# e4s2024/E4S2024

Measured on AMD Instinct MI355X. Metric: 1024x1024 faces/sec (StyleGAN2 regional synthesis, gen_img), higher is better.
Workload: dtype f16+mxfp6x2 (masked 3x3 layers >= 32^2) / bf16x3 (all other layers); 1 GPU; BASELINE configs[1]: StyleGAN2 1024x1024 synthesis from random W+, 12-region masks, batch=4/GPU; batch_per_gpu=4, global_batch=4, parallelism=frames x1, streams_per_gpu=2

## Files before the change

e4s2024_amd/csrc/modconv_upblock_mx.hip:

```cpp
#include "modconv_mx_tile.h"

#ifndef UX_ABL
#define UX_ABL 0
#endif
#ifndef UX_BACK
#define UX_BACK 0
#endif

namespace {

constexpr int UX_OUT = 16;
constexpr int UX_TN = 64, UX_CK = 32;
constexpr int UX_T = UX_OUT / 2 + 2;
constexpr int UX_PW = UX_T + 1;
constexpr int UX_PATCH = UX_PW * UX_PW;
constexpr int UX_NPOS = UX_T * UX_T;
constexpr int UX_EST = 128;
constexpr int UX_ZR = 2 * UX_T, UX_ZS = UX_ZR + 2;
constexpr int UX_NUNIT = 5;
constexpr int UX_U_W16 = 2 * 2 * 2 * UX_TN * 16;
constexpr int UX_U_CLO = 2 * 2 * UX_TN * 16;
constexpr int UX_U_CHI = 2 * 2 * UX_TN * 8;
constexpr int UX_U_SC = 2 * UX_TN * 4;
constexpr int UX_UNITB = 15 * 1024;
constexpr int UX_NPIECE = UX_UNITB / 1024;
static_assert(UX_U_W16 + UX_U_CLO + UX_U_CHI + UX_U_SC <= UX_UNITB, "unit slot");
constexpr int UX_NSLOT = 6;
constexpr int UX_RING = 0;
constexpr int UX_GRP0 = UX_RING + UX_NSLOT * UX_UNITB;
constexpr int UX_A1 = 0;
constexpr int UX_CLO = UX_A1 + 4 * UX_EST * 16;
constexpr int UX_CHI = UX_CLO + 2 * UX_EST * 16;
constexpr int UX_SC = UX_CHI + 2 * UX_EST * 8;
constexpr int UX_SROW = UX_SC + UX_EST * 4;
constexpr int UX_MAX_CIN = 512;
constexpr int UX_EP = UX_SROW + UX_MAX_CIN * 4;
constexpr int UX_RAW = UX_EP + (2 * UX_TN + UX_OUT * UX_OUT) * 4;
constexpr int UX_GRPB = UX_RAW + UX_CK * UX_EST * 4;
constexpr int UX_LDS = UX_GRP0 + 2 * UX_GRPB;
constexpr int UX_ZTB = 16 * UX_ZR * UX_ZS * 4;
static_assert(UX_LDS <= 160 * 1024 && 2 * UX_ZTB <= UX_GRP0 && UX_GRPB % 16 == 0, "LDS plan; the pre-blur tiles overlay the weight ring");

struct UpBlockMxParams {
    float* out;
    const float* x;
    const unsigned char* wmx;
    const float* s;
    const float* d;
    const uint8_t* blocks;
    const int* ctrl;
    const float* blur;
    const float* noise;
    const float* noise_weight;
    const float* act_bias;
    int* flags;
    int noise_bstride, act;
    int bs, cin, cout, h, w, nreg;
    int nbx, nby;
    unsigned perm_mul;
};

__device__ __forceinline__ void ux_wait_vm(int n) {
    switch (n) {
#define UX_CASE(v) case v: E4S_WAIT_VM(v); break;
        UX_CASE(0) UX_CASE(1) UX_CASE(2) UX_CASE(3) UX_CASE(4) UX_CASE(5) UX_CASE(6) UX_CASE(8) UX_CASE(10)
        UX_CASE(16) UX_CASE(17) UX_CASE(18) UX_CASE(19) UX_CASE(20) UX_CASE(21) UX_CASE(22) UX_CASE(24) UX_CASE(26)
        UX_CASE(32) UX_CASE(33) UX_CASE(34) UX_CASE(35) UX_CASE(36) UX_CASE(38) UX_CASE(40)
#undef UX_CASE
        default: E4S_WAIT_VM(0); break;
    }
}

__host__ __device__ constexpr int ux_tap_ky(int u, int d) { return u == 0 ? 0 : u == 1 ? 2 : u == 2 ? 1 : u == 3 ? (d ? 2 : 0) : (d ? 3 : 1); }
__host__ __device__ constexpr int ux_tap_kx(int u, int d) { return u == 0 ? (d ? 2 : 0) : u == 1 ? (d ? 2 : 0) : u == 2 ? (d ? 2 : 0) : 1; }
__host__ __device__ constexpr int ux_parity(int u) { return u == 0 ? 0 : u == 1 ? 0 : u == 2 ? 2 : u == 3 ? 1 : 3; }

__global__ __launch_bounds__(256) void prep_weights_upblock_mx_kernel(unsigned char* __restrict__ dst, const float* __restrict__ weight, int cout, int cin, float scale) {
    const int nchunk = cin / UX_CK, ntile = (cout + UX_TN - 1) / UX_TN;
    const int64_t total = (int64_t)nchunk * ntile * UX_NUNIT * 2 * UX_TN;
    for (int64_t i = (int64_t)blockIdx.x * 256 + threadIdx.x; i < total; i += (int64_t)gridDim.x * 256) {
        int64_t r = i;
        const int n = (int)(r % UX_TN); r /= UX_TN;
        const int half = (int)(r & 1); r >>= 1;
        const int unit = (int)(r % UX_NUNIT); r /= UX_NUNIT;
        const int tile = (int)(r % ntile);
        const int chunk = (int)(r / ntile);
        const int co = tile * UX_TN + n;
        const int ky = ux_tap_ky(unit, half), kx = ux_tap_kx(unit, half);
        unsigned char* slot = dst + (((size_t)chunk * ntile + tile) * UX_NUNIT + unit) * UX_UNITB;
        u32x16 q1, q2;
        float m1 = 0.f, m2 = 0.f;
#pragma unroll
        for (int j = 0; j < 16; ++j) {
            float a = 0.f, b = 0.f;
            if (ky < 3 && co < cout) {
                a = weight[((size_t)co * cin + chunk * UX_CK + 2 * j) * 9 + ky * 3 + kx] * scale;
                b = weight[((size_t)co * cin + chunk * UX_CK + 2 * j + 1) * 9 + ky * 3 + kx] * scale;
            }
            const f16x2 hh = __builtin_convertvector((f32x2){a, b}, f16x2);
            const float ra = (a - (float)hh[0]) * 4096.f, rb = (b - (float)hh[1]) * 4096.f;
            q1[j] = __builtin_bit_cast(unsigned, hh);
            q2[j] = pack_f16_rne(ra, rb);
            m1 = fmaxf(m1, fmaxf(fabsf((float)hh[0]), fabsf((float)hh[1])));
            m2 = fmaxf(m2, fmaxf(fabsf(ra), fabsf(rb)));
        }
        uint4* w16 = reinterpret_cast<uint4*>(slot);
#pragma unroll
        for (int s = 0; s < 4; ++s) w16[(half * 4 + s) * UX_TN + n] = make_uint4(q1[4 * s], q1[4 * s + 1], q1[4 * s + 2], q1[4 * s + 3]);
        auto expo = [](float m) { const unsigned ex = (__builtin_bit_cast(unsigned, m) >> 23) & 0xffu; return ex > 3u ? ex - 2u : 1u; };
        const unsigned e1 = expo(m1), e2 = expo(m2);
        const u32x6 c1 = __builtin_amdgcn_cvt_scalef32_pk32_fp6_f16(__builtin_bit_cast(f16x32, q1), __builtin_bit_cast(float, e1 << 23));
        const u32x6 c2 = __builtin_amdgcn_cvt_scalef32_pk32_fp6_f16(__builtin_bit_cast(f16x32, q2), __builtin_bit_cast(float, e2 << 23));
        uint4* clo = reinterpret_cast<uint4*>(slot + UX_U_W16);
        uint2* chi = reinterpret_cast<uint2*>(slot + UX_U_W16 + UX_U_CLO);
        unsigned* scp = reinterpret_cast<unsigned*>(slot + UX_U_W16 + UX_U_CLO + UX_U_CHI);
        clo[(0 * 2 + half) * UX_TN + n] = make_uint4(c1[0], c1[1], c1[2], c1[3]);
        chi[(0 * 2 + half) * UX_TN + n] = make_uint2(c1[4], c1[5]);
        clo[(1 * 2 + half) * UX_TN + n] = make_uint4(c2[0], c2[1], c2[2], c2[3]);
        chi[(1 * 2 + half) * UX_TN + n] = make_uint2(c2[4], c2[5]);
        const unsigned e2s = e2 > 12u ? e2 - 12u : 0u;
        scp[half * UX_TN + n] = e1 | (e2s << 8);
    }
}

__global__ __launch_bounds__(512, 2) void masked_up_block_mx_kernel(const UpBlockMxParams p) {
    const int npx = p.nbx >> 1;
    const int pr_i = (int)(((unsigned long long)blockIdx.x * p.perm_mul) % gridDim.x);
    const int tyt = pr_i / npx, txp = pr_i - tyt * npx;
    const int b = blockIdx.z;
    if (p.ctrl[2] == 0) return;
    const int reg_a = p.blocks[((size_t)b * p.nby + tyt) * p.nbx + 2 * txp], reg_b = p.blocks[((size_t)b * p.nby + tyt) * p.nbx + 2 * txp + 1];
    if (reg_a >= p.nreg && reg_b >= p.nreg) return;

    extern __shared__ __attribute__((aligned(16))) unsigned char lds[];
    const int tid = threadIdx.x;
    const int lane = tid & 63;
    const int wave = __builtin_amdgcn_readfirstlane(tid >> 6);
    const int grp = wave >> 2, gw = wave & 3;
    const int lt = tid & 255;
    const int txt = 2 * txp + grp;
    const int reg = grp ? reg_b : reg_a;
    const bool live = reg < p.nreg;
    unsigned char* gl = lds + UX_GRP0 + grp * UX_GRPB;
    const int l5 = lane & 31, khalf = lane >> 5;
    const int cot = blockIdx.y, co0 = cot * UX_TN;
    const int ncot = (p.cout + UX_TN - 1) / UX_TN;
    const int hw = p.h * p.w, ho = 2 * p.h, wo = 2 * p.w;
    const int nchunk = p.cin / UX_CK, nunits = nchunk * UX_NUNIT;
    const float* xb = p.x + (size_t)b * p.cin * hw;

    const unsigned char* wbase = p.wmx + (size_t)cot * UX_NUNIT * UX_UNITB;
    auto dma_unit = [&](int g, int slot) __attribute__((always_inline)) {
        const int chunk = g / UX_NUNIT, u = g - chunk * UX_NUNIT;
        const unsigned char* src = wbase + ((size_t)chunk * ncot * UX_NUNIT + u) * UX_UNITB;
#pragma unroll
        for (int k = 0; k < 2; ++k) {
            const int piece = wave + 8 * k;
            if (piece < UX_NPIECE) dma16_asm(src + piece * 1024, (unsigned)(lane * 16), (unsigned)(UX_RING + slot * UX_UNITB + piece * 1024));
        }
    };

    const int pt = (gw & 1) * 64 + lane;
#if UX_BACK & 1
    const bool has_x = gw < 2 && live, has_cv = has_x;
    constexpr int LD_NC = UX_CK;
    const int ld_c0 = 0;
#else
    const bool has_x = live, has_cv = live && (gw >> 1) == grp;
    constexpr int LD_NC = UX_CK / 2;
    const int ld_c0 = (gw >> 1) * LD_NC;
#endif
    const int PCS = wave < 7 ? 2 : 1;
    const int NLD = has_x ? LD_NC : 0;
    auto patch_pixel = [&](bool& in) __attribute__((always_inline)) {
        int t = pt;
        pin_here(t);
        const int se_y = t / UX_PW, se_x = t - se_y * UX_PW;
        const int sgy = tyt * (UX_OUT / 2) - 2 + se_y, sgx = txt * (UX_OUT / 2) - 2 + se_x;
        in = t < UX_PATCH && sgy >= 0 && sgy < p.h && sgx >= 0 && sgx < p.w;
        return in ? (unsigned)(sgy * p.w + sgx) * 4u : 0u;
    };
    const unsigned raw_dst = (unsigned)(UX_GRP0 + grp * UX_GRPB + UX_RAW + (gw & 1) * 64 * 4);
    auto load_x = [&](int chunk) __attribute__((always_inline)) {
        if (has_x) {
            bool in;
            const unsigned goff = patch_pixel(in);
#pragma unroll
            for (int c = 0; c < LD_NC; ++c) dma4_asm(xb + (size_t)(chunk * UX_CK + ld_c0 + c) * hw, goff, raw_dst + (unsigned)((ld_c0 + c) * UX_EST * 4));
        }
    };
    unsigned ovf = 0u;
    auto store_x = [&](int chunk) __attribute__((always_inline)) {
        if (!has_cv) return;
        bool in;
        (void)patch_pixel(in);
        const float4* st = reinterpret_cast<const float4*>(gl + UX_SROW) + chunk * (UX_CK / 4);
        float xr[UX_CK];
        {
            int t = pt;
            pin_here(t);
            const float* raw = reinterpret_cast<const float*>(gl + UX_RAW) + t;
#pragma unroll
            for (int c = 0; c < UX_CK; ++c) xr[c] = raw[c * UX_EST];
        }
        u32x16 q1, q2;
        unsigned m = 0u;
#pragma unroll
        for (int half = 0; half < 2; ++half) {
            float4 s4[4];
#pragma unroll
            for (int k = 0; k < 4; ++k) s4[k] = st[half * 4 + k];
#pragma unroll
            for (int k = 0; k < 4; ++k) {
                const int c4 = half * 4 + k;
                const float a0 = xr[4 * c4] * s4[k].x, a1v = xr[4 * c4 + 1] * s4[k].y, a2v = xr[4 * c4 + 2] * s4[k].z, a3 = xr[4 * c4 + 3] * s4[k].w;
                q1[2 * c4] = pack_f16_rne(a0, a1v);
                q1[2 * c4 + 1] = pack_f16_rne(a2v, a3);
                q2[2 * c4] = resid_pair_f16(xr[4 * c4], s4[k].x, xr[4 * c4 + 1], s4[k].y, q1[2 * c4]);
                q2[2 * c4 + 1] = resid_pair_f16(xr[4 * c4 + 2], s4[k].z, xr[4 * c4 + 3], s4[k].w, q1[2 * c4 + 1]);
                typedef unsigned short u16x2 __attribute__((ext_vector_type(2)));
                u16x2 mm = __builtin_elementwise_max(__builtin_bit_cast(u16x2, m), __builtin_bit_cast(u16x2, q1[2 * c4] & 0x7fff7fffu));
                mm = __builtin_elementwise_max(mm, __builtin_bit_cast(u16x2, q1[2 * c4 + 1] & 0x7fff7fffu));
                m = __builtin_bit_cast(unsigned, mm);
            }
        }
        if (!in) {
#pragma unroll
            for (int j = 0; j < 16; ++j) { q1[j] = 0u; q2[j] = 0u; }
            m = 0u;
        }
        const unsigned mh = (m & 0xffffu) > (m >> 16) ? (m & 0xffffu) : (m >> 16);
        const unsigned e16 = mh >> 10;
        ovf |= e16 >= 31u ? 1u : 0u;
        const unsigned ex = (e16 ? e16 : 1u) + 112u;
        const unsigned e1 = ex > 3u ? ex - 2u : 1u, e2 = ex > 14u ? ex - 13u : 1u;
        const u32x6 c1 = __builtin_amdgcn_cvt_scalef32_pk32_fp6_f16(__builtin_bit_cast(f16x32, q1), __builtin_bit_cast(float, e1 << 23));
        const u32x6 c2 = __builtin_amdgcn_cvt_scalef32_pk32_fp6_f16(__builtin_bit_cast(f16x32, q2), __builtin_bit_cast(float, e2 << 23));
        int t = pt;
        pin_here(t);
        if (t < UX_PATCH) {
            uint4* a1p = reinterpret_cast<uint4*>(gl + UX_A1);
#pragma unroll
            for (int s = 0; s < 4; ++s) a1p[s * UX_EST + t] = make_uint4(q1[4 * s], q1[4 * s + 1], q1[4 * s + 2], q1[4 * s + 3]);
            uint4* clo = reinterpret_cast<uint4*>(gl + UX_CLO);
            uint2* chi = reinterpret_cast<uint2*>(gl + UX_CHI);
            clo[t] = make_uint4(c1[0], c1[1], c1[2], c1[3]);
            chi[t] = make_uint2(c1[4], c1[5]);
            clo[UX_EST + t] = make_uint4(c2[0], c2[1], c2[2], c2[3]);
            chi[UX_EST + t] = make_uint2(c2[4], c2[5]);
            reinterpret_cast<unsigned*>(gl + UX_SC)[t] = e1 | (e2 << 8);
        }
    };

    if (live) {
        const float* srow = p.s + ((size_t)b * p.nreg + reg) * p.cin;
        float* sl = reinterpret_cast<float*>(gl + UX_SROW);
        for (int c = lt; c < p.cin; c += 256) sl[c] = srow[c];
        float* ep_d = reinterpret_cast<float*>(gl + UX_EP);
        float* ep_b = ep_d + UX_TN;
        float* ep_n = ep_b + UX_TN;
        if (lt < UX_TN) {
            const int co = co0 + lt;
            ep_d[lt] = (co < p.cout && p.d) ? p.d[((size_t)b * p.nreg + reg) * p.cout + co] : 1.f;
            ep_b[lt] = (co < p.cout && p.act_bias) ? p.act_bias[co] : 0.f;
        }
        {
            const int ny = tyt * UX_OUT + (lt >> 4), nx = txt * UX_OUT + (lt & 15);
            ep_n[lt] = (p.noise && ny < ho && nx < wo) ? p.noise_weight[0] * p.noise[(size_t)b * p.noise_bstride + (size_t)ny * wo + nx] : 0.f;
        }
    }
    load_x(0);
#pragma unroll
    for (int k = 0; k < UX_NSLOT; ++k)
        if (k < nunits) dma_unit(k, k);
    ux_wait_vm(((nunits < UX_NSLOT ? nunits : UX_NSLOT) - 1) * PCS);
    E4S_LDS_BARRIER();
    store_x(0);
    E4S_LDS_BARRIER();

#if UX_BACK & 2
    const int pos = gw * 32 + l5;
    const bool pos_ok = pos < UX_NPOS;
    const int posc = pos_ok ? pos : UX_NPOS - 1;
    const int pty = posc / UX_T, ptx = posc - pty * UX_T;
    const int xoff = pty * UX_PW + ptx;
#else
    const int lq = l5 >> 2;
    const int li = l5 - 4 * ((lq + 1) >> 1);
    const int lr = li == 15 ? 0 : li / 5, lc = li == 15 ? 5 : li - 5 * lr;
    const int pty = 3 * gw + lr, ptx = 5 * ((0x96 >> lq) & 1) + lc;
    const bool pos_ok = li < 15 && pty < UX_T;
    const int xoff = pty * UX_PW + ptx - (pty >= UX_T ? 32 : 0);
#endif

    f32x16 accs[4][2];
#pragma unroll
    for (int a = 0; a < 4; ++a)
#pragma unroll
        for (int i = 0; i < 2; ++i)
#pragma unroll
            for (int r = 0; r < 16; ++r) accs[a][i][r] = 0.f;

    const unsigned char* wl = lds + UX_RING + (khalf * UX_TN + l5) * 16;
    uint4 xa[2][2], wv[2][2][2];
    auto tap_entry = [&](int u, int d) __attribute__((always_inline)) {
        int xo = xoff;
        pin_here(xo);
        return xo + (1 - (ux_tap_ky(u, d) >> 1)) * UX_PW + (1 - (ux_tap_kx(u, d) >> 1));
    };
    auto read_f16 = [&](int u, int d, int slot) __attribute__((always_inline)) {
        const unsigned char* ws = wl + slot * UX_UNITB;
        const int e = tap_entry(u, d);
#pragma unroll
        for (int j = 0; j < 2; ++j) {
            xa[d][j] = *reinterpret_cast<const uint4*>(gl + UX_A1 + ((2 * j + khalf) * UX_EST + e) * 16);
#pragma unroll
            for (int cb = 0; cb < 2; ++cb) wv[cb][d][j] = *reinterpret_cast<const uint4*>(ws + ((d * 2 + j) * 2 * UX_TN + cb * 32) * 16);
        }
    };
    auto mfma_f16 = [&](int ai, int d) __attribute__((always_inline)) {
#pragma unroll
        for (int j = 0; j < 2; ++j)
#pragma unroll
            for (int cb = 0; cb < 2; ++cb)
                accs[ai][cb] = __builtin_amdgcn_mfma_f32_32x32x16_f16(__builtin_bit_cast(f16x8, wv[cb][d][j]), __builtin_bit_cast(f16x8, xa[d][j]), accs[ai][cb], 0, 0, 0);
    };
    int slot = 0, g = 0;
    if (!(UX_ABL & 1)) read_f16(0, 0, 0);
#pragma unroll 1
    for (int chunk = 0; chunk < ((UX_ABL & 1) ? 0 : nchunk); ++chunk) {
        const bool more = chunk + 1 < nchunk;
        if (more && !(UX_ABL & 4)) load_x(chunk + 1);
#pragma unroll
        for (int u = 0; u < UX_NUNIT; ++u, ++g) {
            const int ai = ux_parity(u);
            const int nslot = slot == UX_NSLOT - 1 ? 0 : slot + 1;
            const bool two = u < UX_NUNIT - 1;
            uint4 calo[2], wclo[2][2];
            uint2 cahi[2], wchi[2][2];
            int scw[2], sca = 0;
            auto read_fp6 = [&](int term) __attribute__((always_inline)) {
                const int ek = (khalf && two) ? tap_entry(u, 1) : tap_entry(u, 0);
                calo[term] = *reinterpret_cast<const uint4*>(gl + UX_CLO + (term * UX_EST + ek) * 16);
                cahi[term] = *reinterpret_cast<const uint2*>(gl + UX_CHI + (term * UX_EST + ek) * 8);
                const unsigned char* wc = lds + UX_RING + slot * UX_UNITB + UX_U_W16 + (khalf * UX_TN + l5) * 16;
                const unsigned char* wh = lds + UX_RING + slot * UX_UNITB + UX_U_W16 + UX_U_CLO + (khalf * UX_TN + l5) * 8;
#pragma unroll
                for (int cb = 0; cb < 2; ++cb) {
                    wclo[cb][1 - term] = *reinterpret_cast<const uint4*>(wc + ((1 - term) * 2 * UX_TN + cb * 32) * 16);
                    wchi[cb][1 - term] = *reinterpret_cast<const uint2*>(wh + ((1 - term) * 2 * UX_TN + cb * 32) * 8);
                }
                if (term == 0) {
                    sca = *reinterpret_cast<const int*>(gl + UX_SC + ek * 4);
                    const unsigned char* wsc = lds + UX_RING + slot * UX_UNITB + UX_U_W16 + UX_U_CLO + UX_U_CHI + (khalf * UX_TN + l5) * 4;
#pragma unroll
                    for (int cb = 0; cb < 2; ++cb) scw[cb] = *reinterpret_cast<const int*>(wsc + cb * 32 * 4);
                }
            };
            if (two) read_f16(u, 1, slot);
            __builtin_amdgcn_sched_barrier(0);
            if (live) mfma_f16(ai, 0);
            __builtin_amdgcn_sched_barrier(0);
            read_fp6(0);
            __builtin_amdgcn_sched_barrier(0);
            if (live && two) mfma_f16(ai, 1);
            __builtin_amdgcn_sched_barrier(0);
            read_fp6(1);
            __builtin_amdgcn_sched_barrier(0);
            if (live) {
#pragma unroll
                for (int cb = 0; cb < 2; ++cb)
                    accs[ai][cb] = __builtin_amdgcn_mfma_scale_f32_32x32x64_f8f6f4(mx_op6(wclo[cb][1], wchi[cb][1]), mx_op6(calo[0], cahi[0]), accs[ai][cb], 2, 2, 1, scw[cb], 0, sca);
            }
            __builtin_amdgcn_sched_barrier(0);
            {
                const int last_req = g - 1 + UX_NSLOT < nunits - 1 ? g - 1 + UX_NSLOT : nunits - 1;
                const int younger = last_req > g + 1 ? last_req - (g + 1) : 0;
                const bool addx = u < UX_NUNIT - 1 && more && !(UX_ABL & 4) && NLD != 0;
                if (younger == UX_NSLOT - 2 && LD_NC == 16) {
                    static_assert(UX_NSLOT == 6, "the literals below are 4 units of 2 / 1 pieces + 16 activation requests");
                    if (addx) { if (PCS == 2) E4S_WAIT_VM(24); else E4S_WAIT_VM(20); }
                    else { if (PCS == 2) E4S_WAIT_VM(8); else E4S_WAIT_VM(4); }
                } else
                    ux_wait_vm(younger * PCS + (addx ? NLD : 0));
            }
            E4S_LDS_BARRIER();
            if (g + UX_NSLOT < nunits) dma_unit(g + UX_NSLOT, slot);
            if (two) {
                read_f16(u + 1, 0, nslot);
                __builtin_amdgcn_sched_barrier(0);
            }
            if (live) {
#pragma unroll
                for (int cb = 0; cb < 2; ++cb)
                    accs[ai][cb] = __builtin_amdgcn_mfma_scale_f32_32x32x64_f8f6f4(mx_op6(wclo[cb][0], wchi[cb][0]), mx_op6(calo[1], cahi[1]), accs[ai][cb], 2, 2, 0, scw[cb], 1, sca);
            }
            slot = nslot;
        }
        if (more) {
            if (!(UX_ABL & 4)) store_x(chunk + 1);
            E4S_LDS_BARRIER();
            read_f16(0, 0, slot);
        }
    }
    E4S_WAIT_VM(0);
    if (p.flags && __builtin_amdgcn_ballot_w64(ovf != 0u) != 0 && lane == 0) { atomicOr(p.flags, 1); atomicAdd(p.flags + 1, 1); }

    if (UX_ABL & 2) { if (accs[0][0][0] == 12345.f) p.out[tid] = accs[1][1][1] + accs[2][0][2] + accs[3][1][3]; return; }
    __syncthreads();
    float* zt = reinterpret_cast<float*>(lds + grp * UX_ZTB);
    const float* ep_d = reinterpret_cast<const float*>(gl + UX_EP);
    const float* ep_b = ep_d + UX_TN;
    const float* ep_n = ep_b + UX_TN;
    float kf[16];
#pragma unroll
    for (int t = 0; t < 16; ++t) kf[t] = p.blur[15 - t];
    const int bx = lt & 15, bco = (lt >> 4) & 7, byg = (lt >> 7) & 1;
    const int oy0 = tyt * UX_OUT + 8 * byg, ox = txt * UX_OUT + bx;
    int nrow = ho - oy0;
    nrow = (!live || nrow < 0) ? 0 : (nrow > 8 ? 8 : nrow);
    const bool col_ok = ox < wo;
    const float* nzp = ep_n + 8 * byg * UX_OUT + bx;
    float nzr[8];
#pragma unroll
    for (int r = 0; r < 8; ++r) nzr[r] = nzp[r * UX_OUT];
    const float neg = p.act ? 0.2f : 1.f, gain = p.act ? 1.41421356237309515f : 1.f;
#pragma unroll
    for (int i = 0; i < 2; ++i) {
#pragma unroll
        for (int gh = 0; gh < 2; ++gh) {
            if (pos_ok && live) {
#pragma unroll
                for (int g2 = 0; g2 < 2; ++g2)
#pragma unroll
                    for (int rr = 0; rr < 4; ++rr) {
                        const int col = 8 * g2 + 4 * khalf + rr;
#pragma unroll
                        for (int ci = 0; ci < 2; ++ci)
                            *reinterpret_cast<float2*>(&zt[(col * UX_ZR + 2 * pty + ci) * UX_ZS + 2 * ptx]) =
                                make_float2(accs[2 * ci][i][4 * (2 * gh + g2) + rr], accs[2 * ci + 1][i][4 * (2 * gh + g2) + rr]);
                    }
            }
            __syncthreads();
            if (nrow > 0 && col_ok) {
#pragma unroll
                for (int c2 = 0; c2 < 2; ++c2) {
                    const int lc = bco + 8 * c2;
                    const int cl = i * 32 + 16 * gh + lc;
                    const int co = co0 + cl;
                    if (co >= p.cout) continue;
                    const float dd = ep_d[cl], bi = ep_b[cl];
                    const float* zc = zt + (lc * UX_ZR + 8 * byg + 1) * UX_ZS + bx + 1;
                    float* orow = p.out + ((size_t)b * p.cout + co) * ho * wo + (size_t)oy0 * wo + ox;
                    float a0 = 0.f, a1 = 0.f, a2 = 0.f, a3;
#pragma unroll
                    for (int zr = 0; zr < 8 + 3; ++zr) {
                        const float* zp = zc + zr * UX_ZS;
                        const float z0 = zp[0], z1 = zp[1], z2 = zp[2], z3 = zp[3];
                        a3 = 0.f;
                        a0 = __builtin_fmaf(z0, kf[12], a0); a1 = __builtin_fmaf(z0, kf[8], a1); a2 = __builtin_fmaf(z0, kf[4], a2); a3 = __builtin_fmaf(z0, kf[0], a3);
                        a0 = __builtin_fmaf(z1, kf[13], a0); a1 = __builtin_fmaf(z1, kf[9], a1); a2 = __builtin_fmaf(z1, kf[5], a2); a3 = __builtin_fmaf(z1, kf[1], a3);
                        a0 = __builtin_fmaf(z2, kf[14], a0); a1 = __builtin_fmaf(z2, kf[10], a1); a2 = __builtin_fmaf(z2, kf[6], a2); a3 = __builtin_fmaf(z2, kf[2], a3);
                        a0 = __builtin_fmaf(z3, kf[15], a0); a1 = __builtin_fmaf(z3, kf[11], a1); a2 = __builtin_fmaf(z3, kf[7], a2); a3 = __builtin_fmaf(z3, kf[3], a3);
                        if (zr >= 3 && zr - 3 < nrow) {
                            float v = __builtin_fmaf(a0, dd, bi) + nzr[zr - 3];
                            v = fmaxf(v, v * neg) * gain;
                            orow[(size_t)(zr - 3) * wo] = v;
                        }
                        a0 = a1; a1 = a2; a2 = a3;
                    }
                }
            }
            __syncthreads();
        }
    }
}

}

extern "C" int e4s_upblock_mx_weight_bytes(int cout, int cin, int64_t* bytes) {
    E4S_REQUIRE(bytes && cout >= 1 && cin >= UX_CK && cin % UX_CK == 0, "upblock_mx_weight_bytes: bad arguments (cin %% 32 == 0)");
    *bytes = (int64_t)(cin / UX_CK) * cdiv(cout, UX_TN) * UX_NUNIT * UX_UNITB;
    return 0;
}

extern "C" int e4s_modconv_prep_weights_upblock_mx(void* dst, const float* weight, int cout, int cin, void* stream) {
    E4S_REQUIRE(dst && weight && cout >= 1 && cin >= UX_CK && cin % UX_CK == 0, "modconv_prep_weights_upblock_mx: bad arguments (cin %% 32 == 0)");
    E4S_REQUIRE(((uintptr_t)dst & 15) == 0, "modconv_prep_weights_upblock_mx: the destination must be 16-byte aligned");
    (void)hipMemsetAsync(dst, 0, (size_t)(cin / UX_CK) * cdiv(cout, UX_TN) * UX_NUNIT * UX_UNITB, (hipStream_t)stream);
    const int64_t total = (int64_t)(cin / UX_CK) * cdiv(cout, UX_TN) * UX_NUNIT * 2 * UX_TN;
    const int grid = (int)(cdiv64(total, 256) < 4096 ? cdiv64(total, 256) : 4096);
    hipLaunchKernelGGL(prep_weights_upblock_mx_kernel, dim3(grid), dim3(256), 0, (hipStream_t)stream, (unsigned char*)dst, weight, cout, cin, 1.0f / sqrtf((float)cin * 9.f));
    return check_launch("modconv_prep_weights_upblock_mx");
}

extern "C" int e4s_masked_upconv_blocks_mx(float* out, const float* x, const void* wmx, int* flags, const float* s, const float* d, const uint8_t* blocks, const int* ctrl,
                                           const float* blur, const float* noise, int noise_bs, const float* noise_weight, const float* act_bias, int act, int bs, int cin,
                                           int cout, int h, int w, int nreg, void* stream) {
    E4S_REQUIRE(out && x && wmx && s && blocks && ctrl && blur, "masked_upconv_blocks_mx: null tensor");
    E4S_REQUIRE(bs >= 0 && bs <= 65535 && cin >= UX_CK && cin % UX_CK == 0 && cin <= UX_MAX_CIN && cout >= 1 && h >= 8 && w >= 8 && (h % 8) == 0 && (w % 8) == 0,
                "masked_upconv_blocks_mx: bad size (cin %% 32 == 0, cin <= 512, h multiple of 8, w multiple of 16)");
    E4S_REQUIRE(w % 16 == 0, "masked_upconv_blocks_mx: the width must be a multiple of 16 (pairs of 16 x 16 output blocks)");
    E4S_REQUIRE(nreg >= 1 && nreg <= E4S_MAX_REGIONS, "masked_upconv_blocks_mx: %d regions (max %d)", nreg, E4S_MAX_REGIONS);
    E4S_REQUIRE(!noise || (noise_weight && (noise_bs == 1 || noise_bs == bs)), "masked_upconv_blocks_mx: noise needs its weight and batch 1 or bs");
    E4S_REQUIRE(((uintptr_t)wmx & 15) == 0, "masked_upconv_blocks_mx: the weights must be 16-byte aligned");
    if (bs == 0) return 0;
    UpBlockMxParams p;
    memset(&p, 0, sizeof(p));
    p.out = out; p.x = x; p.wmx = reinterpret_cast<const unsigned char*>(wmx); p.flags = flags; p.s = s; p.d = d; p.blocks = blocks; p.ctrl = ctrl;
    p.blur = blur; p.noise = noise; p.noise_weight = noise_weight; p.act_bias = act_bias;
    p.noise_bstride = (noise && noise_bs == bs) ? 4 * h * w : 0; p.act = act;
    p.bs = bs; p.cin = cin; p.cout = cout; p.h = h; p.w = w; p.nreg = nreg;
    p.nbx = 2 * w / UX_OUT; p.nby = 2 * h / UX_OUT;
    p.perm_mul = coprime_stride((unsigned)((p.nbx / 2) * p.nby));
    static const hipError_t attr = hipFuncSetAttribute(reinterpret_cast<const void*>(&masked_up_block_mx_kernel), hipFuncAttributeMaxDynamicSharedMemorySize, UX_LDS);
    if (attr != hipSuccess) return fail((int)attr, "masked_upconv_blocks_mx: cannot raise the dynamic LDS limit: %s", hipGetErrorString(attr));
    const dim3 grid((p.nbx / 2) * p.nby, cdiv(cout, UX_TN), bs);
    hipLaunchKernelGGL(masked_up_block_mx_kernel, grid, dim3(512), UX_LDS, (hipStream_t)stream, p);
    return check_launch("masked_upconv_blocks_mx");
}
```

Before: 1527 faces/s.

## Restructure upblock blur epilogue into 4x4 register tiles with vector LDS reads

Result: faster. 1545 faces/s (median of 6 runs) (+1.2%).

```diff
diff --git a/e4s2024_amd/csrc/modconv_upblock_mx.hip b/e4s2024_amd/csrc/modconv_upblock_mx.hip
--- a/e4s2024_amd/csrc/modconv_upblock_mx.hip
+++ b/e4s2024_amd/csrc/modconv_upblock_mx.hip
@@ -1,3 +1,5 @@
+#include <type_traits>
+
 #include "modconv_mx_tile.h"
 
 #ifndef UX_ABL
@@ -16,7 +18,7 @@
 constexpr int UX_PATCH = UX_PW * UX_PW;
 constexpr int UX_NPOS = UX_T * UX_T;
 constexpr int UX_EST = 128;
-constexpr int UX_ZR = 2 * UX_T, UX_ZS = UX_ZR + 2;
+constexpr int UX_ZR = 2 * UX_T;
 constexpr int UX_NUNIT = 5;
 constexpr int UX_U_W16 = 2 * 2 * 2 * UX_TN * 16;
 constexpr int UX_U_CLO = 2 * 2 * UX_TN * 16;
@@ -37,9 +39,18 @@
 constexpr int UX_EP = UX_SROW + UX_MAX_CIN * 4;
 constexpr int UX_RAW = UX_EP + (2 * UX_TN + UX_OUT * UX_OUT) * 4;
 constexpr int UX_GRPB = UX_RAW + UX_CK * UX_EST * 4;
-constexpr int UX_LDS = UX_GRP0 + 2 * UX_GRPB;
-constexpr int UX_ZTB = 16 * UX_ZR * UX_ZS * 4;
-static_assert(UX_LDS <= 160 * 1024 && 2 * UX_ZTB <= UX_GRP0 && UX_GRPB % 16 == 0, "LDS plan; the pre-blur tiles overlay the weight ring");
+constexpr int UX_KF = UX_GRP0 + 2 * UX_GRPB;
+constexpr int UX_LDS = UX_KF + 16 * 4;
+#if UX_BACK & 4
+constexpr int UX_ZP = UX_ZR + 2, UX_ZCP = UX_ZR * UX_ZP;
+#else
+constexpr int UX_ZP = 20, UX_ZCP = 448;
+static_assert(UX_ZP % 4 == 0 && UX_ZP >= UX_ZR && UX_ZCP % 4 == 0 && UX_ZCP >= UX_ZR * UX_ZP && UX_ZCP % 64 == 0 && (12 * UX_ZP) % 64 == 48 && (4 * UX_ZP) % 64 == 16,
+              "pre-blur tile: 16-byte aligned rows, a 16-byte read meets no bank twice");
+#endif
+constexpr int UX_ZTB = 16 * UX_ZCP * 4;
+static_assert(UX_LDS <= 160 * 1024 && 2 * UX_ZTB <= UX_GRP0 && UX_ZTB % 16 == 0 && UX_GRPB % 16 == 0 && UX_EP % 16 == 0,
+              "LDS plan; the pre-blur tiles overlay the weight ring");
 
 struct UpBlockMxParams {
     float* out;
@@ -252,6 +263,9 @@
         }
     };
 
+#if !(UX_BACK & 4)
+    if (tid < 16) reinterpret_cast<float*>(lds + UX_KF)[tid] = p.blur[15 - tid];
+#endif
     if (live) {
         const float* srow = p.s + ((size_t)b * p.nreg + reg) * p.cin;
         float* sl = reinterpret_cast<float*>(gl + UX_SROW);
@@ -413,6 +427,100 @@
     const float* ep_b = ep_d + UX_TN;
     const float* ep_n = ep_b + UX_TN;
     float kf[16];
+    const float neg = p.act ? 0.2f : 1.f, gain = p.act ? 1.41421356237309515f : 1.f;
+    auto put_tile = [&](int i, int gh) __attribute__((always_inline)) {
+        if (pos_ok && live) {
+#pragma unroll
+            for (int g2 = 0; g2 < 2; ++g2)
+#pragma unroll
+                for (int rr = 0; rr < 4; ++rr) {
+                    const int col = 8 * g2 + 4 * khalf + rr;
+#pragma unroll
+                    for (int ci = 0; ci < 2; ++ci)
+                        *reinterpret_cast<float2*>(&zt[col * UX_ZCP + (2 * pty + ci) * UX_ZP + 2 * ptx]) =
+                            make_float2(accs[2 * ci][i][4 * (2 * gh + g2) + rr], accs[2 * ci + 1][i][4 * (2 * gh + g2) + rr]);
+                }
+        }
+    };
+#if !(UX_BACK & 4)
+#pragma unroll
+    for (int t = 0; t < 16; ++t)
+        kf[t] = __builtin_bit_cast(float, __builtin_amdgcn_readfirstlane(reinterpret_cast<const int*>(lds + UX_KF)[t]));
+    constexpr int ER = 4;
+    const int xg = lt & 3, yg = (lt >> 2) & 3, ech = lt >> 4;
+    const int oy0 = tyt * UX_OUT + ER * yg, ox = txt * UX_OUT + 4 * xg;
+    int nrow = ho - oy0;
+    nrow = (!live || nrow < 0) ? 0 : (nrow > ER ? ER : nrow);
+    const bool col_ok = ox < wo;
+    const bool al16 = (reinterpret_cast<uintptr_t>(p.out) & 15) == 0;
+    float4 nzr[ER];
+#pragma unroll
+    for (int r = 0; r < ER; ++r) nzr[r] = *reinterpret_cast<const float4*>(ep_n + (ER * yg + r) * UX_OUT + 4 * xg);
+    auto read16 = [](const float* q) __attribute__((always_inline)) {
+        typedef float f32x4v __attribute__((ext_vector_type(4)));
+        f32x4v v = *reinterpret_cast<const f32x4v*>(q);
+        asm("" : "+v"(v));
+        return v;
+    };
+    auto passes = [&](auto wide) __attribute__((always_inline)) {
+#pragma unroll
+    for (int i = 0; i < 2; ++i) {
+#pragma unroll
+        for (int gh = 0; gh < 2; ++gh) {
+            put_tile(i, gh);
+            __syncthreads();
+            const int cl = i * 32 + 16 * gh + ech;
+            const int co = co0 + cl;
+            if (nrow > 0 && col_ok && co < p.cout) {
+                const float dd = ep_d[cl], bi = ep_b[cl];
+                const float* zc = zt + ech * UX_ZCP + (ER * yg + 1) * UX_ZP + 4 * xg;
+                float* orow = p.out + ((size_t)b * p.cout + co) * ho * wo + (size_t)oy0 * wo + ox;
+                f32x2 pa[4], pb[4];
+#pragma unroll
+                for (int o = 0; o < 4; ++o) { pa[o] = (f32x2){0.f, 0.f}; pb[o] = (f32x2){0.f, 0.f}; }
+#pragma unroll
+                for (int zr = 0; zr < ER + 3; ++zr) {
+                    const auto za = read16(zc + zr * UX_ZP), zb = read16(zc + zr * UX_ZP + 4);
+                    const float z[8] = {za[0], za[1], za[2], za[3], zb[0], zb[1], zb[2], zb[3]};
+#pragma unroll
+                    for (int o = 0; o < 4; ++o) {
+#pragma unroll
+                        for (int u = 0; u < 4; ++u) {
+                            const float zz = z[o + 1 + u];
+                            if (zr == 0) pa[o][0] = __builtin_fmaf(zz, kf[u], pa[o][0]);
+                            else if (zr <= 3) pa[o] = __builtin_elementwise_fma((f32x2){zz, zz}, (f32x2){kf[4 * zr + u], kf[4 * (zr - 1) + u]}, pa[o]);
+                            else if (zr == 4) pa[o][1] = __builtin_fmaf(zz, kf[12 + u], pa[o][1]);
+                            if (zr == 2) pb[o][0] = __builtin_fmaf(zz, kf[u], pb[o][0]);
+                            else if (zr >= 3 && zr <= 5) pb[o] = __builtin_elementwise_fma((f32x2){zz, zz}, (f32x2){kf[4 * (zr - 2) + u], kf[4 * (zr - 3) + u]}, pb[o]);
+                            else if (zr == 6) pb[o][1] = __builtin_fmaf(zz, kf[12 + u], pb[o][1]);
+                        }
+                    }
+                    if (zr >= 3 && zr - 3 < nrow) {
+                        const float nz[4] = {nzr[zr - 3].x, nzr[zr - 3].y, nzr[zr - 3].z, nzr[zr - 3].w};
+                        float v[4];
+#pragma unroll
+                        for (int o = 0; o < 4; ++o) {
+                            const float acc = zr == 3 ? pa[o][0] : zr == 4 ? pa[o][1] : zr == 5 ? pb[o][0] : pb[o][1];
+                            v[o] = __builtin_fmaf(acc, dd, bi) + nz[o];
+                            v[o] = fmaxf(v[o], v[o] * neg) * gain;
+                        }
+                        float* op = orow + (size_t)(zr - 3) * wo;
+                        if (UX_ABL & 8) { if (v[0] == 12345.f) op[0] = v[1] + v[2] + v[3]; }
+                        else if (decltype(wide)::value)
+                            *reinterpret_cast<float4*>(op) = make_float4(v[0], v[1], v[2], v[3]);
+                        else {
+#pragma unroll
+                            for (int o = 0; o < 4; ++o) op[o] = v[o];
+                        }
+                    }
+                }
+            }
+            __syncthreads();
+        }
+    }
+    };
+    if (al16) passes(std::true_type{}); else passes(std::false_type{});
+#else
 #pragma unroll
     for (int t = 0; t < 16; ++t) kf[t] = p.blur[15 - t];
     const int bx = lt & 15, bco = (lt >> 4) & 7, byg = (lt >> 7) & 1;
@@ -424,23 +532,11 @@
     float nzr[8];
 #pragma unroll
     for (int r = 0; r < 8; ++r) nzr[r] = nzp[r * UX_OUT];
-    const float neg = p.act ? 0.2f : 1.f, gain = p.act ? 1.41421356237309515f : 1.f;
 #pragma unroll
     for (int i = 0; i < 2; ++i) {
 #pragma unroll
         for (int gh = 0; gh < 2; ++gh) {
-            if (pos_ok && live) {
-#pragma unroll
-                for (int g2 = 0; g2 < 2; ++g2)
-#pragma unroll
-                    for (int rr = 0; rr < 4; ++rr) {
-                        const int col = 8 * g2 + 4 * khalf + rr;
-#pragma unroll
-                        for (int ci = 0; ci < 2; ++ci)
-                            *reinterpret_cast<float2*>(&zt[(col * UX_ZR + 2 * pty + ci) * UX_ZS + 2 * ptx]) =
-                                make_float2(accs[2 * ci][i][4 * (2 * gh + g2) + rr], accs[2 * ci + 1][i][4 * (2 * gh + g2) + rr]);
-                    }
-            }
+            put_tile(i, gh);
             __syncthreads();
             if (nrow > 0 && col_ok) {
 #pragma unroll
@@ -450,12 +546,12 @@
                     const int co = co0 + cl;
                     if (co >= p.cout) continue;
                     const float dd = ep_d[cl], bi = ep_b[cl];
-                    const float* zc = zt + (lc * UX_ZR + 8 * byg + 1) * UX_ZS + bx + 1;
+                    const float* zc = zt + lc * UX_ZCP + (8 * byg + 1) * UX_ZP + bx + 1;
                     float* orow = p.out + ((size_t)b * p.cout + co) * ho * wo + (size_t)oy0 * wo + ox;
                     float a0 = 0.f, a1 = 0.f, a2 = 0.f, a3;
 #pragma unroll
                     for (int zr = 0; zr < 8 + 3; ++zr) {
-                        const float* zp = zc + zr * UX_ZS;
+                        const float* zp = zc + zr * UX_ZP;
                         const float z0 = zp[0], z1 = zp[1], z2 = zp[2], z3 = zp[3];
                         a3 = 0.f;
                         a0 = __builtin_fmaf(z0, kf[12], a0); a1 = __builtin_fmaf(z0, kf[8], a1); a2 = __builtin_fmaf(z0, kf[4], a2); a3 = __builtin_fmaf(z0, kf[0], a3);
@@ -474,6 +570,7 @@
             __syncthreads();
         }
     }
+#endif
 }
 
 }
```
